# sara-nl/saraGAN

Measured on AMD Instinct MI355X. Metric: 3D volumes/sec/node (G+D step) at 128x128x32, higher is better.
Workload: dtype bf16

## Files before the change

### saragan_amd/csrc/common.h

```cpp
#pragma once
#include <hip/hip_runtime.h>
#include <stdint.h>
#include <mutex>
#include "../../include/saragan_hip.h"

typedef __bf16 bf16_t;
typedef float f32x4 __attribute__((ext_vector_type(4)));
typedef float f32x16 __attribute__((ext_vector_type(16)));
typedef __bf16 bf16x8 __attribute__((ext_vector_type(8)));
typedef __bf16 bf16x4 __attribute__((ext_vector_type(4)));
typedef short s16x4 __attribute__((ext_vector_type(4)));
typedef uint32_t u32x4 __attribute__((ext_vector_type(4)));

#define SG_STORE16_GUARD(v) asm volatile("s_nop 1" ::"v"(v))
typedef uint32_t u32x2 __attribute__((ext_vector_type(2)));

#define SG_LAUNCH_CHECK()                          \
  do {                                             \
    hipError_t e__ = hipGetLastError();            \
    if (e__ != hipSuccess) return (int)e__;        \
  } while (0)

static inline hipStream_t sg_st(sg_stream_t s) { return (hipStream_t)s; }

struct sg_config {
  int fwd_lds, fwd_tg;
  int fwd_v1, fwd_no_pw, fwd_no_dense;
  int fwd_no_v3, fwd_no_v3s, fwd_no_v4, fwd_no_v5, fwd_no_ksplit;
  int fwd3p_16;
  int fwd3s_16;
  int fwd_no_3p;
  int fwd3_gx, fwd3_no_lean;
  int fwd4_gx, fwd4_no_lean, fwd4_no_wres;
  int wgrad_v1, wgrad_no_v3, wgrad_no_lean;
  int wgrad_no_w16;
  int wgrad3l_min_cols;
  int wgrad3l_16;
  int wgrad_v1_blocks;
  int dbg_flags;
  int no_small;
  int deterministic;
  int gemm_ks_model;
  int gemm_k333_maxvox;
  int no_gemm;
};
const sg_config& sg_cfg();

bool sg_gemm_conv_eligible(const sg_conv_shape* s, sg_dtype dt);
size_t sg_gemm_conv_workspace(const sg_conv_shape* s, sg_dtype dt);
int sg_gemm_conv_fwd(const void* x, const void* wp, void* y, const sg_conv_shape* s, const float* bias, int act, float slope,
                     const uint32_t* mask_bits, float mask_slope, uint32_t* sign_out, void* workspace, size_t workspace_bytes,
                     hipStream_t st, bool* used);

bool sg_small_eligible(const sg_conv_shape* s);
bool sg_small_wgrad_eligible(const sg_conv_shape* s);
size_t sg_small_tail_bytes(const sg_conv_shape* s);
size_t sg_small_wgrad_workspace(const sg_conv_shape* s);
int sg_small_pack(const float* w, float coef, int flip, void* tail, const sg_conv_shape* s, sg_dtype dt, hipStream_t st);
int sg_small_fwd(const void* x, const void* tail, void* y, const sg_conv_shape* s, const float* bias, int act, float slope,
                 int pixel_norm, float eps, float* pn_scale, const uint32_t* mask_bits, float mask_slope, uint32_t* sign_out,
                 sg_dtype dt, hipStream_t st);
int sg_small_wgrad(const void* x, const void* dy, float* dw, float* dbias, float coef, void* workspace, size_t workspace_bytes,
// ... 259 lines not shown
```

### saragan_amd/csrc/conv3d.hip

```cpp
#include "common.h"
#include "prof.h"
#include "conv_args.h"

struct PackArgs {
  const float* w;
  void* wp;
  float coef;
  int taps, kd, kh, kw, cin, cout, nchunk, ntile, flip;
};

template <typename T>
__global__ void pack_weights_kernel(PackArgs a) {
  constexpr int CH = sg_traits<T>::CH;
  constexpr int EPL = CH / 2;
  const int64_t total = (int64_t)a.nchunk * a.taps * a.ntile * 64 * EPL;
  T* out = reinterpret_cast<T*>(a.wp);
  for (int64_t i = (int64_t)blockIdx.x * blockDim.x + threadIdx.x; i < total; i += (int64_t)gridDim.x * blockDim.x) {
    int e = (int)(i % EPL);
    int64_t q = i / EPL;
    int lane = (int)(q % 64); q /= 64;
    int nt = (int)(q % a.ntile); q /= a.ntile;
    int tap = (int)(q % a.taps);
    int chunk = (int)(q / a.taps);
    int ci = chunk * CH + (lane >> 5) * EPL + e;
// ... 29 lines not shown
    int lane = (int)(q % 64); q /= 64;
    int nt = (int)(q % a.ntile); q /= a.ntile;
    int tap = (int)(q % a.taps);
    int chunk = (int)(q / a.taps);
    int ci = chunk * CH + (lane >> 5) * EPL + e;
    int co = nt * 32 + (lane & 31);
    float v = 0.f;
    if (ci < a.cin && co < a.cout) {
      v = a.flip ? a.w[((int64_t)(a.taps - 1 - tap) * a.cout + co) * a.cin + ci] : a.w[((int64_t)tap * a.cin + ci) * a.cout + co];
      v *= a.coef;
    }
    out[i] = sg_traits<T>::from_f(v);
  }
}

static inline int conv_nchunk(const sg_conv_shape* s, sg_dtype dt) {
  int ch = dt == SG_BF16 ? 16 : 8;
  return sg_cdiv(s->cin, ch);
}
static inline int conv_ntile(const sg_conv_shape* s) { return sg_cdiv(s->cout, 32); }

static int conv_shape_ok(const sg_conv_shape* s) {
  if (!s) return 0;
  if (s->n < 1 || s->d < 1 || s->h < 1 || s->w < 1 || s->cin < 1 || s->cout < 1) return 0;
  const bool sub = s->kd == 2 && s->kh == 2 && s->kw == 2 && !s->upsample_in;
  if (s->kd < 1 || s->kh < 1 || s->kw < 1 || (!sub && (!(s->kd & 1) || !(s->kh & 1) || !(s->kw & 1)))) return 0;
  if (s->kd > 7 || s->kh > 7 || s->kw > 7) return 0;
  if (s->upsample_in && ((s->d | s->h | s->w) & 1)) return 0;
  return 1;
}

extern "C" size_t sg_conv3d_packed_bytes(const sg_conv_shape* s, sg_dtype dt) {
  if (!conv_shape_ok(s)) return 0;
  return (size_t)conv_nchunk(s, dt) * (s->kd * s->kh * s->kw) * conv_ntile(s) * 1024 + sg_small_tail_bytes(s) + sg_pack16_bytes(s, dt);
}

extern "C" int sg_conv3d_pack_weights(const float* w, float coef, int transpose_flip, void* wp,
                                      const sg_conv_shape* s, sg_dtype dt, sg_stream_t st) {
  if (!conv_shape_ok(s) || !w || !wp) return SG_EINVAL;
  PackArgs a;
  a.w = w; a.wp = wp; a.coef = coef;
  a.kd = s->kd; a.kh = s->kh; a.kw = s->kw; a.taps = s->kd * s->kh * s->kw;
  a.cin = s->cin; a.cout = s->cout; a.nchunk = conv_nchunk(s, dt); a.ntile = conv_ntile(s);
  a.flip = transpose_flip ? 1 : 0;
  int64_t total = (int64_t)a.nchunk * a.taps * a.ntile * 64 * (dt == SG_BF16 ? 8 : 4);
  int blocks = (int)((total + 255) / 256);
  if (blocks > 4096) blocks = 4096;
  if (dt == SG_BF16)
    hipLaunchKernelGGL(pack_weights_kernel<bf16_t>, dim3(blocks), dim3(256), 0, sg_st(st), a);
  else
    hipLaunchKernelGGL(pack_weights_kernel<float>, dim3(blocks), dim3(256), 0, sg_st(st), a);
  SG_LAUNCH_CHECK();
  if (sg_pack16_bytes(s, dt)) {
    void* tail = reinterpret_cast<char*>(wp) + (size_t)a.nchunk * a.taps * a.ntile * 1024;
    return sg_pack16_batch(1, &w, &coef, &a.flip, &tail, s, sg_st(st));
  }
  if (sg_small_tail_bytes(s))
    return sg_small_pack(w, coef, a.flip, reinterpret_cast<char*>(wp) + (size_t)a.nchunk * a.taps * a.ntile * 1024, s, dt, sg_st(st));
  return SG_OK;
}

extern "C" int sg_conv3d_pack_weights_batch(int n, const float* const* w, const float* coef, const int* transpose_flip,
                                            void* const* wp, const sg_conv_shape* shapes, sg_dtype dt, sg_stream_t st) {
  if (n < 0 || (n > 0 && (!w || !coef || !transpose_flip || !wp || !shapes))) return SG_EINVAL;
  if (dt != SG_BF16 && dt != SG_F32) return SG_EINVAL;
  for (int i = 0; i < n; ++i)
    if (!conv_shape_ok(&shapes[i]) || !w[i] || !wp[i]) return SG_EINVAL;
  for (int i0 = 0; i0 < n; i0 += SG_PACK_BATCH) {
    const int m = n - i0 < SG_PACK_BATCH ? n - i0 : SG_PACK_BATCH;
    PackBatchArgs b;
    int64_t most = 0;
    for (int j = 0; j < SG_PACK_BATCH; ++j) {
      const int i = i0 + (j < m ? j : 0);
      const sg_conv_shape* s = &shapes[i];
      PackArgs& a = b.item[j];
      a.w = w[i]; a.wp = wp[i]; a.coef = coef[i];
      a.kd = s->kd; a.kh = s->kh; a.kw = s->kw; a.taps = s->kd * s->kh * s->kw;
      a.cin = s->cin; a.cout = s->cout; a.nchunk = conv_nchunk(s, dt); a.ntile = conv_ntile(s);
      a.flip = transpose_flip[i] ? 1 : 0;
      const int64_t total = (int64_t)a.nchunk * a.taps * a.ntile * 64 * (dt == SG_BF16 ? 8 : 4);
      if (j < m && total > most) most = total;
    }
    int blocks = (int)((most + 255) / 256);
    if (blocks > 256) blocks = 256;
    if (blocks < 1) blocks = 1;
    if (dt == SG_BF16)
      hipLaunchKernelGGL(pack_weights_batch_kernel<bf16_t>, dim3((unsigned)blocks, (unsigned)m), dim3(256), 0, sg_st(st), b);
    else
      hipLaunchKernelGGL(pack_weights_batch_kernel<float>, dim3((unsigned)blocks, (unsigned)m), dim3(256), 0, sg_st(st), b);
    SG_LAUNCH_CHECK();
  }
  constexpr int M16 = 64;
  const float* w16[M16]; float c16[M16]; int f16[M16]; void* d16[M16]; sg_conv_shape s16[M16];
  int n16 = 0;
  for (int i = 0; i < n; ++i) {
    const sg_conv_shape* s = &shapes[i];
    char* tail = reinterpret_cast<char*>(wp[i]) + (size_t)conv_nchunk(s, dt) * (s->kd * s->kh * s->kw) * conv_ntile(s) * 1024;
    int rc = SG_OK;
    if (sg_pack16_bytes(s, dt)) {
      w16[n16] = w[i]; c16[n16] = coef[i]; f16[n16] = transpose_flip[i] ? 1 : 0; d16[n16] = tail; s16[n16] = *s;
      if (++n16 == M16) {
        rc = sg_pack16_batch(n16, w16, c16, f16, d16, s16, sg_st(st));
        n16 = 0;
      }
    } else if (sg_small_tail_bytes(s)) rc = sg_small_pack(w[i], coef[i], transpose_flip[i] ? 1 : 0, tail, s, dt, sg_st(st));
    if (rc != SG_OK) return rc;
  }
  if (n16) return sg_pack16_batch(n16, w16, c16, f16, d16, s16, sg_st(st));
  return SG_OK;
}


template <typename T> struct sg_vec4 { typedef u32x4 type; };
template <> struct sg_vec4<bf16_t> { typedef u32x2 type; };

template <typename T, int MTW, int NTB>
__device__ __forceinline__ void conv_epilogue(f32x16 (&acc)[MTW][NTB], const int64_t (&ooff)[MTW],
                                              const ConvFwdArgs& a, int nt0, int hh) {
  T* y = reinterpret_cast<T*>(a.y);
  const float inv_c = 1.f / (float)a.cout;
#pragma unroll
  for (int mt = 0; mt < MTW; ++mt) {
    float ss = 0.f;
#pragma unroll
    for (int nt = 0; nt < NTB; ++nt) {
#pragma unroll
      for (int i = 0; i < 16; ++i) {
        const int co = (nt0 + nt) * 32 + (i & 3) + 8 * (i >> 2) + 4 * hh;
        float v = acc[mt][nt][i];
        if (a.bias != nullptr && co < a.cout) v += a.bias[co];
        if (a.act) v = fmaxf(v, v * a.slope);
        acc[mt][nt][i] = v;
        ss += v * v;
      }
    }
    if (a.pixel_norm) {
      ss += __shfl_xor(ss, 32);
      const float sc = rsqrtf(ss * inv_c + a.eps);
#pragma unroll
      for (int nt = 0; nt < NTB; ++nt)
#pragma unroll
// ... 2098 lines not shown
    asm volatile("s_waitcnt vmcnt(0)" ::: "memory");
  };

  if (grp == 0) {
    init_acc();
    if (items_mine > 0 && ++cgS == ncg) { cgS = 0; ++kS; if (kS < kmine) enter_tile_S(); }
    for (int q = 0; q < items_max; ++q) {
      stamp();
      if (q < items_mine) mfma_phase(q);
      stamp();
      __syncthreads();
      stamp();
      off_phase(q < items_mine && (q % ncg) == ncg - 1, q + 1, q + 1, HF, NFRAG);
      stamp();
      __syncthreads();
    }
  } else {
    init_acc();
    for (int q = 0; q < items_max; ++q) {
      stamp();
      off_phase(q > 0 && q - 1 < items_mine && ((q - 1) % ncg) == ncg - 1, q, q + 1, 0, HF);
      stamp();
      __syncthreads();
      stamp();
      if (q < items_mine) mfma_phase(q);
      stamp();
      __syncthreads();
    }
    if (items_mine > 0 && items_mine == items_max) off_phase(true, items_mine, items_max, 0, 0);
    else if (items_mine > 0) {  }
  }
}

template <int EPI>
static int launch_fwd5_inst(const ConvFwdArgs& a, unsigned gx, unsigned gy, size_t lds, hipStream_t st) {
  auto kern = conv_fwd5_kernel<EPI>;
  SG_ALLOW_160K_LDS(kern);
  hipLaunchKernelGGL(kern, dim3(gx, gy), dim3(512), lds, st, a);
  return SG_OK;
}

static int launch_fwd5(ConvFwdArgs& a, const sg_conv_shape* s, hipStream_t st, bool* used) {
  *used = false;
  if (s->upsample_in || s->kd != 3 || s->kh != 3 || s->kw != 3 || a.os == 2 || a.tap_d || a.tap_h || a.tap_w) return SG_OK;
  if ((s->cin % 16) != 0 || (s->cout % 64) != 0 || a.pool == 1) return SG_OK;
  if (a.pool && ((s->h | s->w) & 1 || a.pixel_norm || a.mask_bits)) return SG_OK;
  if (a.pixel_norm && (a.mask_bits || a.ntile != 2)) return SG_OK;
  if (a.mask_bits && a.sign_out) return SG_OK;
  a.g = sg_make_geom(s, 256, true);
  const sg_tile_geom& g = a.g;
  if (g.TN != 1 || g.TW != 32 || (g.TH & 1) || g.TD * g.TH * g.TW != 256 || g.HD > 127 || g.HH > 127 || g.HW > 127) return SG_OK;
  const int64_t ntiles = (int64_t)g.nTn * g.nTd * g.nTh * g.nTw;
  const int ny = a.ntile / 2;
  int gx = (256 / ny) / 8 * 8;
  if (gx < 8) gx = 8;
  if (ntiles >= (1 << 24) || ntiles < 2 * gx) return SG_OK;
  {
    const int64_t svox = (int64_t)s->d * s->h * s->w;
    if (svox * s->cin * 2 >= (1ll << 31) || svox * s->cout * 2 >= (1ll << 31) || svox * a.ntile * 4 >= (1ll << 31)) return SG_OK;
  }
  const int hv = g.HD * g.HH * g.HW;
  if (sg_cdiv(hv * 2, 64) > 32) return SG_OK;
  a.G = 1;
  a.rs = 32;
  a.xbytes = hv * 32;
  a.wbytes = 27 * 2 * 1024;
  a.wres = 0;
  const size_t lds = 2ull * a.xbytes + 2ull * a.wbytes + 256;
  if (lds > 160 * 1024) return SG_OK;
  a.ntiles = (int)ntiles;
  a.vec_in = 1;
  a.vec_out = 1;
  const int epi = (a.sign_out ? SG_EP_SIGN : 0) | (a.mask_bits ? SG_EP_MASK : 0) | (a.pixel_norm ? SG_EP_PN : 0) |
                  (a.pool ? SG_EP_POOL : 0);
  int rc = SG_OK;
  switch (epi) {
    case 0: rc = launch_fwd5_inst<0>(a, (unsigned)gx, (unsigned)ny, lds, st); break;
    case SG_EP_POOL: rc = launch_fwd5_inst<SG_EP_POOL>(a, (unsigned)gx, (unsigned)ny, lds, st); break;
    case SG_EP_SIGN | SG_EP_POOL: rc = launch_fwd5_inst<SG_EP_SIGN | SG_EP_POOL>(a, (unsigned)gx, (unsigned)ny, lds, st); break;
    case SG_EP_SIGN: rc = launch_fwd5_inst<SG_EP_SIGN>(a, (unsigned)gx, (unsigned)ny, lds, st); break;
    case SG_EP_MASK: rc = launch_fwd5_inst<SG_EP_MASK>(a, (unsigned)gx, (unsigned)ny, lds, st); break;
    case SG_EP_PN: rc = launch_fwd5_inst<SG_EP_PN>(a, (unsigned)gx, (unsigned)ny, lds, st); break;
    case SG_EP_PN | SG_EP_SIGN: rc = launch_fwd5_inst<SG_EP_PN | SG_EP_SIGN>(a, (unsigned)gx, (unsigned)ny, lds, st); break;
    default: return SG_OK;
  }
  if (rc != SG_OK) return rc;
  SG_KNAME("conv_fwd5<bf16,2,2,3,3,3>");
  SG_LAUNCH_CHECK();
  *used = true;
  return SG_OK;
}

template <typename T>
__device__ __forceinline__ float sg_packed_w(const char* wp, int ntile, int cin_j, int cout_c) {
  constexpr int CH = sg_traits<T>::CH, ES = (int)sizeof(T);
  const int chunk = cin_j / CH, hh = (cin_j % CH) / (CH / 2), e = cin_j % (CH / 2);
  const char* frag = wp + ((int64_t)(chunk * ntile + (cout_c >> 5)) << 10);
  return sg_traits<T>::to_f(*reinterpret_cast<const T*>(frag + ((cout_c & 31) + 32 * hh) * 16 + e * ES));
}

template <typename T, int CIN>
__global__ __launch_bounds__(256) void pw_fwd_small_cin_kernel(ConvFwdArgs a, int64_t nvox) {
  constexpr int E = 16 / (int)sizeof(T);
  const int P = a.cout / E;
  const int p = threadIdx.x % P;
  const int c0 = p * E;
  const char* wp = reinterpret_cast<const char*>(a.wp);
  float w[CIN][E], b[E];
// ... 483 lines not shown
```

### saragan_amd/csrc/conv3w.hip

```cpp
#include "common.h"
#include "prof.h"
#include "conv_args.h"

typedef __attribute__((address_space(3))) void* lds_ptr3w_t;
typedef const __attribute__((address_space(1))) void* gbl_ptr3w_t;

namespace {

constexpr int W3_NFRAG = 54;
constexpr int W3_WBYTES = W3_NFRAG * 1024;
constexpr int W3_HROWS = 4 * 34;
constexpr int W3_HALO = W3_HROWS * 64;
constexpr int W3_HOFF = W3_WBYTES;
constexpr int W3_BOFF = W3_HOFF + 8 * W3_HALO;
constexpr int W3_POFF = W3_BOFF + 128;
constexpr int W3_MOFF = W3_POFF + 64;
constexpr int W3_AOFF = W3_MOFF + 128;
constexpr int W3_LDS = W3_MOFF + 128;
constexpr int W3_LDS_PWB = W3_AOFF + 8 * 4096;
static_assert(W3_LDS_PWB <= 160 * 1024, "LDS budget");
constexpr int W3_NPIECE = 9;
static_assert(W3_LDS <= 160 * 1024, "LDS budget");
#ifndef W3_PFW
#define W3_PFW 3
// ... 640 lines not shown
    if (E.j >= nitems) break;
    sg_kloop3w<2>::run(acc, xa, wl);
    stamp();
    SG_W3_OFF(2);
    if (E.j >= nitems) break;
  }
#undef SG_W3_OFF
  if constexpr (PWB) {
    const f32x4 fin[4] = {pwacc[0], pwacc[1], pwacc[2], pwacc[3]};
#pragma unroll
    for (int ch = 0; ch < 2; ++ch)
#pragma unroll
      for (int i = 0; i < 4; ++i) {
        float sw = fin[ch][i], sb = fin[2 + ch][i];
#pragma unroll
        for (int m = 1; m < 16; m <<= 1) {
          sw += __shfl_xor(sw, m);
          sb += __shfl_xor(sb, m);
        }
        if (v16 == 0) {
          float* row = a.pw_part + (size_t)(blockIdx.x * 8 + w8) * 64;
          row[16 * ch + 4 * q4 + i] = sw;
          row[32 + 16 * ch + 4 * q4 + i] = sb;
        }
      }
  }
}

struct Pack16Args {
  const float* w;
  bf16_t* out;
  float coef;
  int cin, cout, ngi, flip;
};
constexpr int SG_PACK16_BATCH = 32;
struct Pack16Batch {
  Pack16Args item[SG_PACK16_BATCH];
};
__global__ void pack_weights16_batch_kernel(Pack16Batch b) {
  const Pack16Args& a = b.item[blockIdx.y];
  const int ntile = a.cout >> 5;
  const int total = ntile * 27 * a.ngi * 2 * 64 * 8;
  for (int i = blockIdx.x * blockDim.x + threadIdx.x; i < total; i += gridDim.x * blockDim.x) {
    const int e = i & 7, lane = (i >> 3) & 63;
    int f = i >> 9;
    const int ch = f & 1;
    f >>= 1;
    const int gi = f % a.ngi;
    f /= a.ngi;
    const int tap = f % 27, nt = f / 27;
    const int co = 32 * nt + 16 * ch + (lane & 15), ci = 32 * gi + 8 * (lane >> 4) + e;
    const float v = !a.flip ? a.w[((int64_t)tap * a.cin + ci) * a.cout + co]
                            : a.w[((int64_t)(26 - tap) * a.cout + co) * a.cin + ci];
    a.out[i] = (bf16_t)(v * a.coef);
  }
}

__global__ __launch_bounds__(1024) void pw_part_final_kernel(const float* __restrict__ part, int rows, float* __restrict__ dw,
                                                             float* __restrict__ dbias, float coef) {
  __shared__ float red[16][64];
  const int col = threadIdx.x & 63, rg = threadIdx.x >> 6;
  float s8[8] = {0.f, 0.f, 0.f, 0.f, 0.f, 0.f, 0.f, 0.f};
  int b = rg;
  for (; b + 7 * 16 < rows; b += 8 * 16) {
#pragma unroll
    for (int u = 0; u < 8; ++u) s8[u] += part[(size_t)(b + u * 16) * 64 + col];
  }
  for (int u = 0; b < rows; b += 16, ++u) s8[u & 7] += part[(size_t)b * 64 + col];
  red[rg][col] = ((s8[0] + s8[1]) + (s8[2] + s8[3])) + ((s8[4] + s8[5]) + (s8[6] + s8[7]));
  __syncthreads();
  if (rg == 0) {
    float t = 0.f;
#pragma unroll
    for (int g = 0; g < 16; ++g) t += red[g][col];
    if (col < 32) { if (dw) dw[col] = coef * t; }
    else if (dbias) dbias[col - 32] = t;
  }
}

template <int EPI>
int launch_fwd3w_inst(const Fwd3wArgs& fa, unsigned gx, hipStream_t st) {
  auto kern = conv_fwd3w_kernel<EPI>;
  SG_ALLOW_160K_LDS(kern);
  hipLaunchKernelGGL(kern, dim3(gx, (unsigned)fa.a.ntile), dim3(512), (EPI & SG_EP_PWB) ? W3_LDS_PWB : W3_LDS, st, fa);
  return SG_OK;
}

}

size_t sg_pack16_bytes(const sg_conv_shape* s, sg_dtype dt) {
  if (dt != SG_BF16 || s->kd != 3 || s->kh != 3 || s->kw != 3 || (s->cout & 31) || s->cout < 32) return 0;
  if (!((s->cin == 64 && s->cout == 32) || s->cin == 32)) return 0;
  return (size_t)(s->cout >> 5) * 27 * (s->cin >> 5) * 2 * 1024;
}

int sg_pack16_batch(int n, const float* const* w, const float* coef, const int* flip, void* const* dst, const sg_conv_shape* shapes,
                    hipStream_t st) {
  for (int i0 = 0; i0 < n; i0 += SG_PACK16_BATCH) {
    const int m = n - i0 < SG_PACK16_BATCH ? n - i0 : SG_PACK16_BATCH;
    Pack16Batch b;
    for (int j = 0; j < SG_PACK16_BATCH; ++j) {
      const int i = i0 + (j < m ? j : 0);
      Pack16Args& p = b.item[j];
      p.w = w[i]; p.out = reinterpret_cast<bf16_t*>(dst[i]); p.coef = coef[i];
      p.cin = shapes[i].cin; p.cout = shapes[i].cout; p.ngi = shapes[i].cin >> 5; p.flip = flip[i] ? 1 : 0;
    }
    hipLaunchKernelGGL(pack_weights16_batch_kernel, dim3(54, (unsigned)m), dim3(256), 0, st, b);
    SG_LAUNCH_CHECK();
  }
  return SG_OK;
}

int sg_pw_wgrad_finalize(const float* part, int rows, float* dw, float* dbias, float coef, hipStream_t st) {
  if (!dw && !dbias) return SG_OK;
  hipLaunchKernelGGL(pw_part_final_kernel, dim3(1), dim3(1024), 0, st, part, rows, dw, dbias, coef);
  SG_LAUNCH_CHECK();
  return SG_OK;
}

int sg_launch_fwd3w(ConvFwdArgs& a, const sg_conv_shape* s, hipStream_t st, bool* used, int* pw_rows) {
  *used = false;
  *pw_rows = 0;
  if (s->kd != 3 || s->kh != 3 || s->kw != 3 || s->cin != 32 || (s->cout & 31) || a.xcs != 32 || a.xco != 0) return SG_OK;
  if (s->upsample_in || a.in_mask || a.addend) return SG_OK;
  if (s->d < 2 || s->h < 8 || (s->w % 32) != 0) return SG_OK;
  if (a.pool && ((a.pool != 1 && a.pool != 3) || (s->d & 1) || (a.pool == 3 && ((s->h | s->w) & 1)) || a.pixel_norm || a.pnb_y || (a.mask_bits && (a.sign_out || a.bias || a.act)))) return SG_OK;
  if (a.pixel_norm && (a.mask_bits || a.ntile != 1 || a.pnb_y)) return SG_OK;
  if (a.mask_bits && a.sign_out) return SG_OK;
  if (a.pnb_y && (a.ntile != 1 || !a.mask_bits || a.sign_out || a.bias || a.act || !a.pnb_scale)) return SG_OK;
  if (a.rgb_out && (a.ntile != 1 || !a.rgb_w || a.pool || a.mask_bits || a.pnb_y || !a.pixel_norm || !a.sign_out)) return SG_OK;
  if (a.pw_x && (a.ntile != 1 || !a.pw_wmat || !a.pw_part || !a.mask_bits || a.pool || a.pnb_y || a.rgb_out || a.pixel_norm ||
                 a.sign_out || a.bias || a.act)) return SG_OK;
  {
    const int64_t svox = (int64_t)s->d * s->h * s->w;
    if (svox * 64 >= (1ll << 31) || svox * s->cout * 2 >= (1ll << 31) || svox * a.ntile * 4 >= (1ll << 31)) return SG_OK;
  }
  Fwd3wArgs fa;
  fa.a = a;
// ... 50 lines not shown
```

### saragan_amd/csrc/conv_args.h

```cpp
#pragma once
#include "common.h"

struct ConvFwdArgs {
  const void* x;
  const void* wp;
  void* y;
  const float* bias;
  float* pn_scale;
  const uint32_t* mask_bits;
  uint32_t* sign_out;
  float mask_slope;
  sg_tile_geom g;
  int cin, cout, taps, kh, kw;
  int nchunk, ntile;
  int G, TG;
  int rs;
  int xbytes;
  sg_fastdiv fnp;
  int sshift, rshift;
  int wbytes, ntiles;
  int wres;
  int lean;
  int tap_d, tap_h, tap_w;
  int xcs, xco;
  const float* addend;
  const void* pnb_y;
  const float* pnb_scale;
  const uint32_t* in_mask;
  float in_mask_slope, in_gain;
  int in_mask_nw;
  const float* rgb_w;
  const float* rgb_bias;
  void* rgb_out;
  const void* pw_x;
  const float* pw_wmat;
  void* pw_dx;
  float* pw_part;
  int pool;
  int os, oa, ob, oc;
  unsigned long long* dbg;
  int dbg_flags;
  int vec_in, vec_out;
  int act, pixel_norm;
  float slope, eps;
};

enum : int { SG_EP_SIGN = 1, SG_EP_MASK = 2, SG_EP_PN = 4, SG_EP_POOL = 8, SG_EP_PNB = 16,
              SG_EP_RGB = 32, SG_EP_PWB = 128, SG_EP_POOL3 = 256   };

int sg_launch_fwd3p(ConvFwdArgs& a, const sg_conv_shape* s, hipStream_t st, bool* used);
int sg_launch_fwd3w(ConvFwdArgs& a, const sg_conv_shape* s, hipStream_t st, bool* used, int* pw_rows);
constexpr int SG_PW_PART_ROWS = 2048;
int sg_pw_wgrad_finalize(const float* part, int rows, float* dw, float* dbias, float coef, hipStream_t st);
size_t sg_pack16_bytes(const sg_conv_shape* s, sg_dtype dt);
int sg_pack16_batch(int n, const float* const* w, const float* coef, const int* flip, void* const* dst, const sg_conv_shape* shapes,
                    hipStream_t st);
```

### saragan_amd/csrc/prof.hip

```cpp
#include "prof.h"
#include <mutex>
#include <vector>
#include <string.h>
#include <stdlib.h>
#include <atomic>

namespace {
struct Rec { int kind; sg_conv_shape shape; int dtype; hipEvent_t e0, e1; bool ok; const char* name; };
std::mutex g_mu;
bool g_on = false;
bool g_filter = false;
int g_fkind = 0;
sg_conv_shape g_fshape;
std::vector<Rec> g_recs;
const char* kVersion = "saragan_hip 0.4 (gfx950)";
}

bool sg_prof_on() { return g_on; }
thread_local const char* sg_tls_kernel = "";

namespace {
std::atomic<const sg_config*> g_cfg{nullptr};
int env_int(const char* name, int dflt) {
  const char* v = getenv(name);
  return v && *v ? atoi(v) : dflt;
}
const sg_config* read_config() {
  sg_config* c = new sg_config;
  c->fwd_lds = env_int("SG_FWD_LDS", 80 * 1024);
  c->fwd_tg = env_int("SG_FWD_TG", 0);
  c->fwd_v1 = env_int("SG_FWD_V1", 0);
  c->fwd_no_pw = env_int("SG_FWD_NO_PW", 0);
  c->fwd_no_dense = env_int("SG_FWD_NO_DENSE", 0);
  c->fwd_no_v3 = env_int("SG_FWD_NO_V3", 0);
  c->fwd_no_v3s = env_int("SG_FWD_NO_V3S", 0);
  c->wgrad_no_lean = env_int("SG_WGRAD_NO_LEAN", 0);
  c->wgrad_no_w16 = env_int("SG_WGRAD_NO_W16", 0);
  c->wgrad3l_16 = env_int("SG_WGRAD3L_16", 0);
  c->wgrad3l_min_cols = env_int("SG_WGRAD3L_MIN_COLS", 0);
  c->wgrad_v1_blocks = env_int("SG_WGRAD_V1_BLOCKS", 0);
  c->fwd_no_v4 = env_int("SG_FWD_NO_V4", 0);
  c->fwd_no_v5 = env_int("SG_FWD_NO_V5", 0);
  c->fwd_no_ksplit = env_int("SG_FWD_NO_KSPLIT", 0);
  c->fwd_no_3p = env_int("SG_FWD_NO_3P", 0);
  c->fwd3p_16 = env_int("SG_FWD3P_16", 1);
  c->fwd3s_16 = env_int("SG_FWD3S_16", 1);
  c->fwd3_gx = env_int("SG_FWD3_GX", 0);
  c->fwd3_no_lean = env_int("SG_FWD3_NO_LEAN", 0);
  c->fwd4_gx = env_int("SG_FWD4_GX", 0);
  c->fwd4_no_lean = env_int("SG_FWD4_NO_LEAN", 0);
  c->fwd4_no_wres = env_int("SG_FWD4_NO_WRES", 0);
  c->wgrad_v1 = env_int("SG_WGRAD_V1", 0);
  c->wgrad_no_v3 = env_int("SG_WGRAD_NO_V3", 0);
  c->dbg_flags = env_int("SG_DBG_FLAGS", 0);
  c->no_small = env_int("SG_NO_SMALL", 0);
  c->deterministic = env_int("SG_DETERMINISTIC", 0);
  c->no_gemm = env_int("SG_NO_GEMM", 0);
  c->gemm_ks_model = env_int("SG_GEMM_KS_MODEL", 0);
  c->gemm_k333_maxvox = env_int("SG_GEMM_K333_MAXVOX", 8192);
  return c;
}
}

const sg_config& sg_cfg() {
  const sg_config* c = g_cfg.load(std::memory_order_acquire);
  if (c == nullptr) {
    std::lock_guard<std::mutex> lk(g_mu);
    c = g_cfg.load(std::memory_order_acquire);
    if (c == nullptr) {
      c = read_config();
      g_cfg.store(c, std::memory_order_release);
    }
  }
  return *c;
}

extern "C" int sg_config_reload(void) {
  std::lock_guard<std::mutex> lk(g_mu);
// ... 96 lines not shown
```

Before: 615.1.

## Add fwd5p conv kernel using 16x16x32 bf16 MFMA with new packed weight layout

Adds a new 3x3x3 forward convolution kernel variant (fwd5p) that uses v_mfma_f32_16x16x32_bf16 with a fully unrolled, statically checked LDS-read/MFMA schedule, and pairs taps so that 27 taps map to 13 pairs plus a tail. A new weight packing format (kind 1) is added to the batch packing kernel and stored after the pack16 tail, and the packed buffer size grows to hold it. By default (SG_FWD5_16=1) the new kernel replaces fwd5 for eligible shapes without pixel norm, with the aim of raising MFMA throughput and reducing LDS traffic. This adds extra weight packing work and storage, and a complex hand-scheduled kernel whose lgkmcnt accounting is fragile.

Result: no change. 620.6 (median of 6 runs) (+0.9%).

```diff
diff --git a/saragan_amd/csrc/common.h b/saragan_amd/csrc/common.h
--- a/saragan_amd/csrc/common.h
+++ b/saragan_amd/csrc/common.h
@@ -28,6 +28,7 @@
   int fwd_v1, fwd_no_pw, fwd_no_dense;
   int fwd_no_v3, fwd_no_v3s, fwd_no_v4, fwd_no_v5, fwd_no_ksplit;
   int fwd3p_16;
+  int fwd5_16;
   int fwd3s_16;
   int fwd_no_3p;
   int fwd3_gx, fwd3_no_lean;
diff --git a/saragan_amd/csrc/conv3d.hip b/saragan_amd/csrc/conv3d.hip
--- a/saragan_amd/csrc/conv3d.hip
+++ b/saragan_amd/csrc/conv3d.hip
@@ -85,7 +85,8 @@
 
 extern "C" size_t sg_conv3d_packed_bytes(const sg_conv_shape* s, sg_dtype dt) {
   if (!conv_shape_ok(s)) return 0;
-  return (size_t)conv_nchunk(s, dt) * (s->kd * s->kh * s->kw) * conv_ntile(s) * 1024 + sg_small_tail_bytes(s) + sg_pack16_bytes(s, dt);
+  return (size_t)conv_nchunk(s, dt) * (s->kd * s->kh * s->kw) * conv_ntile(s) * 1024 + sg_small_tail_bytes(s) + sg_pack16_bytes(s, dt) +
+         sg_pack5_bytes(s, dt);
 }
 
 extern "C" int sg_conv3d_pack_weights(const float* w, float coef, int transpose_flip, void* wp,
@@ -104,9 +105,17 @@
   else
     hipLaunchKernelGGL(pack_weights_kernel<float>, dim3(blocks), dim3(256), 0, sg_st(st), a);
   SG_LAUNCH_CHECK();
-  if (sg_pack16_bytes(s, dt)) {
-    void* tail = reinterpret_cast<char*>(wp) + (size_t)a.nchunk * a.taps * a.ntile * 1024;
-    return sg_pack16_batch(1, &w, &coef, &a.flip, &tail, s, sg_st(st));
+  if (sg_pack16_bytes(s, dt) || sg_pack5_bytes(s, dt)) {
+    char* tail = reinterpret_cast<char*>(wp) + (size_t)a.nchunk * a.taps * a.ntile * 1024;
+    const float* w2[2] = {w, w};
+    const float c2[2] = {coef, coef};
+    const int f2[2] = {a.flip, a.flip};
+    const sg_conv_shape s2[2] = {*s, *s};
+    void* d2[2];
+    int k2[2], m = 0;
+    if (sg_pack16_bytes(s, dt)) { d2[m] = tail; k2[m++] = 0; }
+    if (sg_pack5_bytes(s, dt)) { d2[m] = tail + sg_pack16_bytes(s, dt); k2[m++] = 1; }
+    return sg_pack16_batch(m, w2, c2, f2, d2, s2, k2, sg_st(st));
   }
   if (sg_small_tail_bytes(s))
     return sg_small_pack(w, coef, a.flip, reinterpret_cast<char*>(wp) + (size_t)a.nchunk * a.taps * a.ntile * 1024, s, dt, sg_st(st));
@@ -143,23 +152,29 @@
       hipLaunchKernelGGL(pack_weights_batch_kernel<float>, dim3((unsigned)blocks, (unsigned)m), dim3(256), 0, sg_st(st), b);
     SG_LAUNCH_CHECK();
   }
-  constexpr int M16 = 64;
-  const float* w16[M16]; float c16[M16]; int f16[M16]; void* d16[M16]; sg_conv_shape s16[M16];
+  constexpr int M16 = 80;
+  const float* w16[M16]; float c16[M16]; int f16[M16]; void* d16[M16]; sg_conv_shape s16[M16]; int k16[M16];
   int n16 = 0;
   for (int i = 0; i < n; ++i) {
     const sg_conv_shape* s = &shapes[i];
     char* tail = reinterpret_cast<char*>(wp[i]) + (size_t)conv_nchunk(s, dt) * (s->kd * s->kh * s->kw) * conv_ntile(s) * 1024;
     int rc = SG_OK;
-    if (sg_pack16_bytes(s, dt)) {
-      w16[n16] = w[i]; c16[n16] = coef[i]; f16[n16] = transpose_flip[i] ? 1 : 0; d16[n16] = tail; s16[n16] = *s;
-      if (++n16 == M16) {
-        rc = sg_pack16_batch(n16, w16, c16, f16, d16, s16, sg_st(st));
-        n16 = 0;
+    const size_t b16 = sg_pack16_bytes(s, dt), b5 = sg_pack5_bytes(s, dt);
+    if (b16 || b5) {
+      for (int kind = 0; kind < 2; ++kind) {
+        if (!(kind ? b5 : b16)) continue;
+        w16[n16] = w[i]; c16[n16] = coef[i]; f16[n16] = transpose_flip[i] ? 1 : 0; d16[n16] = tail + (kind ? b16 : 0); s16[n16] = *s;
+        k16[n16] = kind;
+        if (++n16 == M16) {
+          rc = sg_pack16_batch(n16, w16, c16, f16, d16, s16, k16, sg_st(st));
+          n16 = 0;
+          if (rc != SG_OK) return rc;
+        }
       }
     } else if (sg_small_tail_bytes(s)) rc = sg_small_pack(w[i], coef[i], transpose_flip[i] ? 1 : 0, tail, s, dt, sg_st(st));
     if (rc != SG_OK) return rc;
   }
-  if (n16) return sg_pack16_batch(n16, w16, c16, f16, d16, s16, sg_st(st));
+  if (n16) return sg_pack16_batch(n16, w16, c16, f16, d16, s16, k16, sg_st(st));
   return SG_OK;
 }
 
@@ -2324,6 +2339,415 @@
   }
 }
 
+struct sg_unrolled_k5p {
+  static constexpr int NS = 14, NR = 8;
+  static constexpr int need(int m) { return 4 + m / 4; }
+  static constexpr int issued_next(int s, int m) { return s + 1 < NS ? (m == 0 ? 0 : m == 1 ? 2 : 4) + m / 4 : 0; }
+  static constexpr bool waits(int m) { return (m & 3) == 0; }
+  static constexpr int younger(int s, int m) { return NR - 1 - need(m) + issued_next(s, m); }
+  static constexpr bool counts_ok() {
+    for (int s = 0; s < NS; ++s)
+      for (int m = 0; m < 16; ++m) if (younger(s, m) < 0 || younger(s, m) > 15) return false;
+    return younger(0, 0) == 3 && younger(0, 4) == 7 && younger(0, 12) == 7 && younger(NS - 1, 12) == 0;
+  }
+  static constexpr int NA = 30;
+
+  template <int S, int B>
+  static __device__ __forceinline__ void rdb(u32x4 (&bfr)[2][4], const int (&xa)[NA]) {
+    if constexpr (S < NS - 1)
+      asm volatile("ds_read_b128 %0, %1 offset:%2" : "=v"(bfr[S & 1][B]) : "v"(xa[2 * S + (B >> 1)]), "n"((B & 1) * 512));
+    else
+      asm volatile("ds_read_b128 %0, %1" : "=v"(bfr[S & 1][B]) : "v"(xa[26 + B]));
+  }
+  template <int S, int CG>
+  static __device__ __forceinline__ void rda(u32x4 (&afr)[4], int wl, int wlh) {
+    if constexpr (S < NS - 1)
+      asm volatile("ds_read_b128 %0, %1 offset:%2" : "=v"(afr[CG]) : "v"(wl), "n"((S * 4 + CG) << 10));
+    else
+      asm volatile("ds_read_b128 %0, %1 offset:%2" : "=v"(afr[CG]) : "v"(wlh), "n"(((NS - 1) * 4 << 10) + CG * 512));
+  }
+  static __device__ __forceinline__ void mfma(f32x4& c, const u32x4& a_, const u32x4& b_) {
+    asm volatile("v_mfma_f32_16x16x32_bf16 %0, %1, %2, %0" : "+v"(c) : "v"(a_), "v"(b_));
+  }
+  template <int S, int M>
+  static __device__ __forceinline__ void step(f32x4 (&acc)[2][2][4], u32x4 (&afr)[4], u32x4 (&bfr)[2][4], const int (&xa)[NA], int wl,
+                                              int wlh) {
+    if constexpr (S < NS) {
+      if constexpr (waits(M)) {
+        SG_WAIT_LGKM(younger(S, M));
+        __builtin_amdgcn_sched_barrier(0);
+      }
+      mfma(acc[(M >> 1) & 1][M & 1][M >> 2], afr[M >> 2], bfr[S & 1][M & 3]);
+      if constexpr (S + 1 < NS) {
+        if constexpr (M < 2) {
+          rdb<S + 1, 2 * M>(bfr, xa);
+          rdb<S + 1, 2 * M + 1>(bfr, xa);
+        }
+        if constexpr ((M & 3) == 3) rda<S + 1, (M >> 2)>(afr, wl, wlh);
+      }
+      if constexpr (M < 15) step<S, M + 1>(acc, afr, bfr, xa, wl, wlh);
+      else step<S + 1, 0>(acc, afr, bfr, xa, wl, wlh);
+    }
+  }
+  static __device__ __forceinline__ void run(f32x4 (&acc)[2][2][4], const int (&xa)[NA], int wl, int wlh) {
+    u32x4 afr[4], bfr[2][4];
+    SG_KLOOP_BEGIN();
+    rdb<0, 0>(bfr, xa); rdb<0, 1>(bfr, xa); rdb<0, 2>(bfr, xa); rdb<0, 3>(bfr, xa);
+    rda<0, 0>(afr, wl, wlh); rda<0, 1>(afr, wl, wlh); rda<0, 2>(afr, wl, wlh); rda<0, 3>(afr, wl, wlh);
+    step<0, 0>(acc, afr, bfr, xa, wl, wlh);
+    asm volatile("s_nop 7\n\ts_nop 7\n\ts_nop 3"
+                 : "+v"(acc[0][0][0]), "+v"(acc[0][0][1]), "+v"(acc[0][0][2]), "+v"(acc[0][0][3]),
+                   "+v"(acc[0][1][0]), "+v"(acc[0][1][1]), "+v"(acc[0][1][2]), "+v"(acc[0][1][3]),
+                   "+v"(acc[1][0][0]), "+v"(acc[1][0][1]), "+v"(acc[1][0][2]), "+v"(acc[1][0][3]),
+                   "+v"(acc[1][1][0]), "+v"(acc[1][1][1]), "+v"(acc[1][1][2]), "+v"(acc[1][1][3]));
+    SG_KLOOP_END();
+  }
+};
+static_assert(sg_unrolled_k5p::counts_ok(), "a needed read is issued too late, or lgkmcnt (a 4-bit counter) would overflow");
+
+template <int EPI>
+__global__ __launch_bounds__(512) void conv_fwd5p_kernel(ConvFwdArgs a) {
+  extern __shared__ __attribute__((aligned(16))) char smem[];
+  constexpr int ES = 2, EPP = 8, NFRAG = 54, HF = NFRAG / 2;
+  constexpr uint32_t DEAD = 0x80000000u;
+  constexpr bool SIGN = (EPI & SG_EP_SIGN) != 0, MASK = (EPI & SG_EP_MASK) != 0, PN = (EPI & SG_EP_PN) != 0;
+  constexpr bool POOL = (EPI & SG_EP_POOL) != 0;
+  const sg_tile_geom& g = a.g;
+  const int tid = threadIdx.x, lane = tid & 63;
+  const int wave8 = __builtin_amdgcn_readfirstlane(tid >> 6);
+  const int grp = wave8 >> 2, wave = wave8 & 3;
+  const int q4 = lane >> 4, v16 = (lane & 15) ^ ((lane & 8) ? 0 : 4);
+  const int xmine = grp * a.xbytes, wbase = 2 * a.xbytes;
+  float* bias_lds = reinterpret_cast<float*>(smem + 2 * a.xbytes + 2 * a.wbytes);
+  const int zoff = 2 * a.xbytes + 2 * a.wbytes + 256;
+  const int nt0 = blockIdx.y * 2;
+  const int ncg = a.nchunk, cout = a.cout, ntile = a.ntile, cin = a.cin;
+  const int D = g.D, H = g.H, W = g.W;
+
+  const int xg = blockIdx.x & 7, slot = blockIdx.x >> 3;
+  const int per_x = gridDim.x >> 3;
+  const int cpx = (a.ntiles + 7) >> 3;
+  const int t_begin = xg * cpx;
+  const int t_end = min(a.ntiles, t_begin + cpx);
+  const int first = t_begin + slot;
+  const int K = first < t_end ? (t_end - first + per_x - 1) / per_x : 0;
+  const int kmine = (K + 1 - grp) >> 1;
+  const int items_mine = kmine * ncg;
+  const int items_max = ((K + 1) >> 1) * ncg;
+
+  int xa[sg_unrolled_k5p::NA];
+  int tcoord[2];
+  {
+    const int tsel = q4 >> 1, half = q4 & 1;
+#pragma unroll
+    for (int mt = 0; mt < 2; ++mt) {
+      const int q = wave * 2 + mt;
+      const int th = q % g.TH, td = q / g.TH;
+      tcoord[mt] = (th << 8) | (td << 16);
+      const int lrow = (td * g.HH + th) * g.HW + v16;
+      auto addr_of = [&](int row) { return xmine + row * 32 + ((half ^ ((row >> 3) & 1)) << 4); };
+      auto shift_of = [&](int t) { return ((t / 9) * g.HH + (t / 3) % 3) * g.HW + t % 3; };
+#pragma unroll
+      for (int p = 0; p < 13; ++p) xa[2 * p + mt] = addr_of(lrow + (tsel ? shift_of(2 * p + 1) : shift_of(2 * p)));
+#pragma unroll
+      for (int vh = 0; vh < 2; ++vh) xa[26 + 2 * mt + vh] = tsel ? zoff : addr_of(lrow + shift_of(26) + 16 * vh);
+    }
+  }
+  const int hv = g.HD * g.HH * g.HW;
+  constexpr int MAXIT = 8;
+  uint32_t relb[MAXIT];
+  int crd[MAXIT];
+#pragma unroll
+  for (int k = 0; k < MAXIT; ++k) {
+    const int it = (wave + 4 * k) * 64 + lane;
+    const int row = it >> 1;
+    const int sl = (it & 1) ^ ((row >> 3) & 1);
+    uint32_t q = sg_div((uint32_t)row, g.fHW);
+    const int hw = (int)(row - q * g.HW);
+    uint32_t q2 = sg_div(q, g.fHH);
+    const int hh_ = (int)(q - q2 * g.HH), hd = (int)q2;
+    relb[k] = row < hv ? (uint32_t)((((hd * H + hh_) * W + hw) * cin + sl * EPP) * ES) : 0xC0000000u;
+    crd[k] = row < hv ? (hw | (hh_ << 8) | (hd << 16)) : 0x7F7F7F7F;
+  }
+  const int64_t svox = (int64_t)D * H * W;
+  const int64_t xsb = svox * cin * ES, ysb = (POOL ? svox >> 2 : svox) * cout * ES, wsb = svox * ntile * 4, psb = svox * 4;
+  auto rsrc_of = [&](const void* base, int64_t sample_bytes, int n0) {
+    return __builtin_amdgcn_make_buffer_rsrc(const_cast<char*>(reinterpret_cast<const char*>(base)) + n0 * sample_bytes, 0,
+                                             (int)sample_bytes, 0x00020000);
+  };
+  const __amdgpu_buffer_rsrc_t rw = __builtin_amdgcn_make_buffer_rsrc(const_cast<void*>(a.wp), 0, 0x7FFFFFFF, 0x00020000);
+
+  int kS = 0, cgS = 0;
+  __amdgpu_buffer_rsrc_t rxS;
+  uint32_t vk[MAXIT];
+  auto enter_tile_S = [&]() {
+    const sg_tile_origin o = sg_tile_of(g, (uint32_t)(first + (2 * kS + grp) * per_x));
+    rxS = rsrc_of(a.x, xsb, o.n0);
+    const int tile_off = (((o.d0 - 1) * H + (o.h0 - 1)) * W + (o.w0 - 1)) * cin * ES;
+    const int lo_w = max(0, 1 - o.w0), hi_w = min(g.HW, W + 1 - o.w0) - 1;
+    const int lo_h = max(0, 1 - o.h0), hi_h = min(g.HH, H + 1 - o.h0) - 1;
+    const int lo_d = max(0, 1 - o.d0), hi_d = min(g.HD, D + 1 - o.d0) - 1;
+    const uint32_t lo = (uint32_t)(lo_w | (lo_h << 8) | (lo_d << 16));
+    const uint32_t hi = (uint32_t)(hi_w | (hi_h << 8) | (hi_d << 16)) | 0x808080u;
+#pragma unroll
+    for (int k = 0; k < MAXIT; ++k) {
+      const uint32_t c_ = (uint32_t)crd[k] & 0xFFFFFFu;
+      const uint32_t t1 = (c_ | 0x808080u) - lo, t2 = hi - c_;
+      vk[k] = (t1 & t2 & 0x808080u) == 0x808080u ? relb[k] + (uint32_t)tile_off : DEAD;
+    }
+  };
+  auto stage_halo = [&]() {
+    const uint32_t soff = (uint32_t)(cgS * 32);
+#pragma unroll
+    for (int k = 0; k < MAXIT; ++k)
+      if ((wave + 4 * k) * 64 < hv * 2 && crd[k] != 0x7F7F7F7F)
+        __builtin_amdgcn_raw_ptr_buffer_load_lds(rxS, (lds_ptr_t)(smem + xmine + (wave + 4 * k) * 1024), 16, vk[k], soff, 0, 0);
+  };
+  auto stage_slab = [&](int j, int f0, int f1, int w, int nw) {
+    const int cg = j % ncg;
+    char* dst = smem + wbase + (j & 1) * a.wbytes;
+    const uint32_t cbase = (uint32_t)((cg * (int)gridDim.y + (int)blockIdx.y) * NFRAG) << 10;
+    for (int f = f0 + w; f < f1; f += nw)
+      __builtin_amdgcn_raw_ptr_buffer_load_lds(rw, (lds_ptr_t)(dst + (f << 10)), 16, (uint32_t)(lane * 16), cbase + ((uint32_t)f << 10), 0, 0);
+  };
+  int kE = 0;
+  __amdgpu_buffer_rsrc_t ryE, rsE, rmE, rpE;
+  uint32_t vox[2][2];
+  uint32_t pvox = DEAD;
+  auto enter_tile_E = [&]() {
+    const sg_tile_origin o = sg_tile_of(g, (uint32_t)(first + (2 * kE + grp) * per_x));
+    ryE = rsrc_of(a.y, ysb, o.n0);
+    if (SIGN) rsE = rsrc_of(a.sign_out, wsb, o.n0);
+    if (MASK) rmE = rsrc_of(a.mask_bits, wsb, o.n0);
+    if (PN) rpE = rsrc_of(a.pn_scale, psb, o.n0);
+#pragma unroll
+    for (int mt = 0; mt < 2; ++mt) {
+      const int tc = tcoord[mt];
+      const int d = o.d0 + (tc >> 16), h = o.h0 + ((tc >> 8) & 255);
+#pragma unroll
+      for (int vh = 0; vh < 2; ++vh) {
+        const int w = o.w0 + 16 * vh + v16;
+        vox[mt][vh] = (d < D && h < H && w < W) ? (uint32_t)((d * H + h) * W + w) : DEAD;
+      }
+      if (POOL && mt == 0) {
+        const int w = o.w0 + 2 * ((v16 >> 1) + 8 * (v16 & 1));
+        pvox = (d < D && h < H && w < W) ? (uint32_t)((d * (H >> 1) + (h >> 1)) * (W >> 1) + (w >> 1)) : DEAD;
+      }
+    }
+  };
+  uint32_t mbn[2][2][2] = {{{0u, 0u}, {0u, 0u}}, {{0u, 0u}, {0u, 0u}}};
+  auto request_mask = [&]() {
+    if constexpr (MASK) {
+#pragma unroll
+      for (int mt = 0; mt < 2; ++mt)
+#pragma unroll
+        for (int vh = 0; vh < 2; ++vh)
+#pragma unroll
+          for (int nt = 0; nt < 2; ++nt)
+            mbn[mt][vh][nt] = __builtin_amdgcn_raw_buffer_load_b32(rmE, (kE < kmine && vox[mt][vh] != DEAD) ? (vox[mt][vh] * (uint32_t)ntile + nt0 + nt) * 4u : DEAD, 0, 0);
+    }
+  };
+
+  if (tid < 64) {
+    const int co = nt0 * 32 + tid;
+    bias_lds[tid] = (a.bias != nullptr && co < cout) ? a.bias[co] : 0.f;
+  } else if (tid < 68) {
+    reinterpret_cast<uint32_t*>(smem + zoff)[tid - 64] = 0u;
+  }
+  if (items_max > 0) stage_slab(0, 0, NFRAG, wave8, 8);
+  if (items_mine > 0) {
+    enter_tile_S();
+    enter_tile_E();
+    request_mask();
+    if (grp == 0) stage_halo();
+  }
+  asm volatile("s_waitcnt vmcnt(0)" ::: "memory");
+  __syncthreads();
+
+  const int wl0 = wbase + lane * 16, wlh0 = wbase + (lane & 31) * 16;
+  const float inv_c = 1.f / (float)cout;
+  const float slope = a.act ? a.slope : 1.f;
+  const uint32_t cb = (uint32_t)((q4 & 1) * 16 + (q4 >> 1) * 8);
+  f32x4 acc[2][2][4];
+  auto init_acc = [&]() {
+#pragma unroll
+    for (int cg = 0; cg < 4; ++cg) {
+      const f32x4 b4 = *reinterpret_cast<const f32x4*>(bias_lds + cg * 16 + 4 * q4);
+#pragma unroll
+      for (int mt = 0; mt < 2; ++mt)
+#pragma unroll
+        for (int vh = 0; vh < 2; ++vh) acc[mt][vh][cg] = b4;
+    }
+    asm volatile("" : "+v"(acc[0][0][0]), "+v"(acc[0][0][1]), "+v"(acc[0][0][2]), "+v"(acc[0][0][3]),
+                      "+v"(acc[0][1][0]), "+v"(acc[0][1][1]), "+v"(acc[0][1][2]), "+v"(acc[0][1][3]),
+                      "+v"(acc[1][0][0]), "+v"(acc[1][0][1]), "+v"(acc[1][0][2]), "+v"(acc[1][0][3]),
+                      "+v"(acc[1][1][0]), "+v"(acc[1][1][1]), "+v"(acc[1][1][2]), "+v"(acc[1][1][3]));
+  };
+  int dbgi = 0;
+  auto stamp = [&]() {
+    if (a.dbg != nullptr && blockIdx.x == 8 && blockIdx.y == 0 && lane == 0 && wave == 0 && dbgi < 120)
+      a.dbg[grp * 128 + dbgi] = __builtin_amdgcn_s_memtime();
+    ++dbgi;
+  };
+  auto mfma_phase = [&](int q) { sg_unrolled_k5p::run(acc, xa, wl0 + (q & 1) * a.wbytes, wlh0 + (q & 1) * a.wbytes); };
+  auto quad_sum = [](float v) {
+    const auto r1 = __builtin_amdgcn_permlane16_swap(__float_as_uint(v), __float_as_uint(v), false, false);
+    const float s1 = __uint_as_float(r1[0]) + __uint_as_float(r1[1]);
+    const auto r2 = __builtin_amdgcn_permlane32_swap(__float_as_uint(s1), __float_as_uint(s1), false, false);
+    return __uint_as_float(r2[0]) + __uint_as_float(r2[1]);
+  };
+  auto store_tile = [&](const float (&lo)[4], const float (&hi)[4], const __amdgpu_buffer_rsrc_t& rs, uint32_t voff) {
+    const uint32_t a0 = sg_pack_bf16(lo[0], lo[1]), a1 = sg_pack_bf16(lo[2], lo[3]);
+    const uint32_t b0 = sg_pack_bf16(hi[0], hi[1]), b1 = sg_pack_bf16(hi[2], hi[3]);
+    const auto s0 = __builtin_amdgcn_permlane16_swap(a0, b0, false, false);
+    const auto s1 = __builtin_amdgcn_permlane16_swap(a1, b1, false, false);
+    u32x4 out;
+    out[0] = s0[0]; out[1] = s1[0]; out[2] = s0[1]; out[3] = s1[1];
+    __builtin_amdgcn_raw_buffer_store_b128(out, rs, voff, 0, 0);
+    SG_STORE16_GUARD(out);
+  };
+
+  auto off_phase = [&](bool closes, int qn, int js, int f0, int f1) {
+    if (qn < items_mine) stage_halo();
+    if (js < items_max) stage_slab(js, f0, f1, wave, 4);
+    __builtin_amdgcn_sched_barrier(0);
+    stamp();
+    if (closes) {
+      uint32_t part[2][4] = {{0u, 0u, 0u, 0u}, {0u, 0u, 0u, 0u}};
+#pragma unroll
+      for (int mt = 0; mt < 2; ++mt)
+#pragma unroll
+        for (int vh = 0; vh < 2; ++vh) {
+          f32x4(&t)[4] = acc[mt][vh];
+          const bool ok = vox[mt][vh] != DEAD;
+          if (slope != 1.f) {
+#pragma unroll
+            for (int cg = 0; cg < 4; ++cg)
+#pragma unroll
+              for (int i = 0; i < 4; ++i) t[cg][i] = sg_lrelu(t[cg][i], slope);
+          }
+          if (PN) {
+            float ss = 0.f;
+#pragma unroll
+            for (int cg = 0; cg < 4; ++cg)
+#pragma unroll
+              for (int i = 0; i < 4; ++i) ss += t[cg][i] * t[cg][i];
+            ss = quad_sum(ss);
+            const float sc = rsqrtf(ss * inv_c + a.eps);
+#pragma unroll
+            for (int cg = 0; cg < 4; ++cg)
+#pragma unroll
+              for (int i = 0; i < 4; ++i) t[cg][i] *= sc;
+            if (a.pn_scale != nullptr)
+              __builtin_amdgcn_raw_buffer_store_b32(__float_as_uint(sc), rpE, (ok && q4 == 0) ? vox[mt][vh] * 4u : DEAD, 0, 0);
+          }
+#pragma unroll
+          for (int nt = 0; nt < 2; ++nt) {
+            if (SIGN) {
+              uint32_t b = 0u;
+#pragma unroll
+              for (int ch = 0; ch < 2; ++ch)
+#pragma unroll
+                for (int i = 0; i < 4; ++i) b |= (__float_as_uint(t[2 * nt + ch][i]) >> 31) << (16 * ch + i);
+              part[nt][2 * mt + vh] = b << (4 * q4);
+            }
+            if (MASK) {
+              const uint32_t wsh = mbn[mt][vh][nt] >> (4 * q4);
+              const float sm1 = a.mask_slope - 1.f;
+#pragma unroll
+              for (int ch = 0; ch < 2; ++ch)
+#pragma unroll
+                for (int i = 0; i < 4; ++i) {
+                  const int t_ = ((int)(wsh << (31 - (16 * ch + i)))) >> 31;
+                  t[2 * nt + ch][i] += __uint_as_float((uint32_t)t_ & __float_as_uint(t[2 * nt + ch][i] * sm1));
+                }
+            }
+            if constexpr (!POOL) {
+              const float lo[4] = {t[2 * nt][0], t[2 * nt][1], t[2 * nt][2], t[2 * nt][3]};
+              const float hi[4] = {t[2 * nt + 1][0], t[2 * nt + 1][1], t[2 * nt + 1][2], t[2 * nt + 1][3]};
+              store_tile(lo, hi, ryE, ok ? (vox[mt][vh] * (uint32_t)cout + (uint32_t)((nt0 + nt) * 32) + cb) * 2u : DEAD);
+            }
+          }
+        }
+      if constexpr (SIGN) {
+        const uint32_t sv = q4 == 0 ? vox[0][0] : q4 == 1 ? vox[0][1] : q4 == 2 ? vox[1][0] : vox[1][1];
+#pragma unroll
+        for (int nt = 0; nt < 2; ++nt) {
+          const auto r01 = __builtin_amdgcn_permlane16_swap(part[nt][0], part[nt][1], false, false);
+          const auto r23 = __builtin_amdgcn_permlane16_swap(part[nt][2], part[nt][3], false, false);
+          const auto rr = __builtin_amdgcn_permlane32_swap(r01[0] | r01[1], r23[0] | r23[1], false, false);
+          __builtin_amdgcn_raw_buffer_store_b32(rr[0] | rr[1], rsE, sv != DEAD ? (sv * (uint32_t)ntile + nt0 + nt) * 4u : DEAD, 0, 0);
+        }
+      }
+      if constexpr (POOL) {
+#pragma unroll
+        for (int nt = 0; nt < 2; ++nt) {
+          float m[2][4];
+#pragma unroll
+          for (int ch = 0; ch < 2; ++ch)
+#pragma unroll
+            for (int i = 0; i < 4; ++i) {
+              const float c0 = acc[0][0][2 * nt + ch][i] + acc[1][0][2 * nt + ch][i];
+              const float c1 = acc[0][1][2 * nt + ch][i] + acc[1][1][2 * nt + ch][i];
+              const float u0 = c0 + __uint_as_float((uint32_t)__builtin_amdgcn_update_dpp(0, (int)__float_as_uint(c0), 0xB1, 0xF, 0xF, true));
+              const float u1 = c1 + __uint_as_float((uint32_t)__builtin_amdgcn_update_dpp(0, (int)__float_as_uint(c1), 0xB1, 0xF, 0xF, true));
+              m[ch][i] = ((v16 & 1) ? u1 : u0) * 0.25f;
+            }
+          store_tile(m[0], m[1], ryE, pvox != DEAD ? (pvox * (uint32_t)cout + (uint32_t)((nt0 + nt) * 32) + cb) * 2u : DEAD);
+        }
+      }
+      ++kE;
+      if (kE < kmine) enter_tile_E();
+      request_mask();
+      init_acc();
+    }
+    if (qn < items_mine) {
+      if (++cgS == ncg) {
+        cgS = 0;
+        ++kS;
+        if (kS < kmine) enter_tile_S();
+      }
+    }
+    asm volatile("s_waitcnt vmcnt(0)" ::: "memory");
+  };
+
+  if (grp == 0) {
+    init_acc();
+    if (items_mine > 0 && ++cgS == ncg) { cgS = 0; ++kS; if (kS < kmine) enter_tile_S(); }
+    for (int q = 0; q < items_max; ++q) {
+      stamp();
+      if (q < items_mine) mfma_phase(q);
+      stamp();
+      __syncthreads();
+      stamp();
+      off_phase(q < items_mine && (q % ncg) == ncg - 1, q + 1, q + 1, HF, NFRAG);
+      stamp();
+      __syncthreads();
+    }
+  } else {
+    init_acc();
+    for (int q = 0; q < items_max; ++q) {
+      stamp();
+      off_phase(q > 0 && q - 1 < items_mine && ((q - 1) % ncg) == ncg - 1, q, q + 1, 0, HF);
+      stamp();
+      __syncthreads();
+      stamp();
+      if (q < items_mine) mfma_phase(q);
+      stamp();
+      __syncthreads();
+    }
+    if (items_mine > 0 && items_mine == items_max) off_phase(true, items_mine, items_max, 0, 0);
+  }
+}
+
+template <int EPI>
+static int launch_fwd5p_inst(const ConvFwdArgs& a, unsigned gx, unsigned gy, size_t lds, hipStream_t st) {
+  auto kern = conv_fwd5p_kernel<EPI>;
+  SG_ALLOW_160K_LDS(kern);
+  hipLaunchKernelGGL(kern, dim3(gx, gy), dim3(512), lds, st, a);
+  return SG_OK;
+}
+
 template <int EPI>
 static int launch_fwd5_inst(const ConvFwdArgs& a, unsigned gx, unsigned gy, size_t lds, hipStream_t st) {
   auto kern = conv_fwd5_kernel<EPI>;
@@ -2366,6 +2790,22 @@
   const int epi = (a.sign_out ? SG_EP_SIGN : 0) | (a.mask_bits ? SG_EP_MASK : 0) | (a.pixel_norm ? SG_EP_PN : 0) |
                   (a.pool ? SG_EP_POOL : 0);
   int rc = SG_OK;
+  const size_t lds16 = lds + 16;
+  const bool use16 = sg_cfg().fwd5_16 == 2 || (sg_cfg().fwd5_16 == 1 && !a.pixel_norm);
+  if (use16 && sg_pack5_bytes(s, SG_BF16) && lds16 <= 160 * 1024) {
+    ConvFwdArgs b = a;
+    b.wp = reinterpret_cast<const char*>(a.wp) + (size_t)a.nchunk * a.taps * a.ntile * 1024 + sg_pack16_bytes(s, SG_BF16);
+    switch (epi) {
+      case 0: rc = launch_fwd5p_inst<0>(b, (unsigned)gx, (unsigned)ny, lds16, st); break;
+      case SG_EP_POOL: rc = launch_fwd5p_inst<SG_EP_POOL>(b, (unsigned)gx, (unsigned)ny, lds16, st); break;
+      case SG_EP_SIGN | SG_EP_POOL: rc = launch_fwd5p_inst<SG_EP_SIGN | SG_EP_POOL>(b, (unsigned)gx, (unsigned)ny, lds16, st); break;
+      case SG_EP_SIGN: rc = launch_fwd5p_inst<SG_EP_SIGN>(b, (unsigned)gx, (unsigned)ny, lds16, st); break;
+      case SG_EP_MASK: rc = launch_fwd5p_inst<SG_EP_MASK>(b, (unsigned)gx, (unsigned)ny, lds16, st); break;
+      case SG_EP_PN: rc = launch_fwd5p_inst<SG_EP_PN>(b, (unsigned)gx, (unsigned)ny, lds16, st); break;
+      case SG_EP_PN | SG_EP_SIGN: rc = launch_fwd5p_inst<SG_EP_PN | SG_EP_SIGN>(b, (unsigned)gx, (unsigned)ny, lds16, st); break;
+      default: return SG_OK;
+    }
+  } else
   switch (epi) {
     case 0: rc = launch_fwd5_inst<0>(a, (unsigned)gx, (unsigned)ny, lds, st); break;
     case SG_EP_POOL: rc = launch_fwd5_inst<SG_EP_POOL>(a, (unsigned)gx, (unsigned)ny, lds, st); break;
diff --git a/saragan_amd/csrc/conv3w.hip b/saragan_amd/csrc/conv3w.hip
--- a/saragan_amd/csrc/conv3w.hip
+++ b/saragan_amd/csrc/conv3w.hip
@@ -696,13 +696,41 @@
   bf16_t* out;
   float coef;
   int cin, cout, ngi, flip;
+  int kind;
 };
-constexpr int SG_PACK16_BATCH = 32;
+constexpr int SG_PACK16_BATCH = 80;
 struct Pack16Batch {
   Pack16Args item[SG_PACK16_BATCH];
 };
+static_assert(sizeof(Pack16Batch) <= 4096, "kernel arguments");
+constexpr int SG_PACK5_PAIRS = 13, SG_PACK5_SLAB = SG_PACK5_PAIRS * 4 * 512 + 4 * 256;
 __global__ void pack_weights16_batch_kernel(Pack16Batch b) {
   const Pack16Args& a = b.item[blockIdx.y];
+  if (a.kind == 1) {
+    const int nb = a.cout >> 6;
+    const int total = (a.cin >> 4) * nb * SG_PACK5_SLAB;
+    for (int i = blockIdx.x * blockDim.x + threadIdx.x; i < total; i += gridDim.x * blockDim.x) {
+      const int slab = i / SG_PACK5_SLAB, r = i - slab * SG_PACK5_SLAB;
+      const int chunk = slab / nb, blk = slab - chunk * nb;
+      const int e = r & 7;
+      int lane, cg, tap;
+      if (r < SG_PACK5_PAIRS * 4 * 512) {
+        lane = (r >> 3) & 63;
+        cg = (r >> 9) & 3;
+        tap = 2 * (r >> 11) + (lane >> 5);
+      } else {
+        const int r2 = r - SG_PACK5_PAIRS * 4 * 512;
+        lane = (r2 >> 3) & 31;
+        cg = r2 >> 8;
+        tap = 26;
+      }
+      const int co = 64 * blk + 16 * cg + (lane & 15), ci = 16 * chunk + 8 * ((lane >> 4) & 1) + e;
+      const float v = !a.flip ? a.w[((int64_t)tap * a.cin + ci) * a.cout + co]
+                              : a.w[((int64_t)(26 - tap) * a.cout + co) * a.cin + ci];
+      a.out[i] = (bf16_t)(v * a.coef);
+    }
+    return;
+  }
   const int ntile = a.cout >> 5;
   const int total = ntile * 27 * a.ngi * 2 * 64 * 8;
   for (int i = blockIdx.x * blockDim.x + threadIdx.x; i < total; i += gridDim.x * blockDim.x) {
@@ -758,8 +786,14 @@
   return (size_t)(s->cout >> 5) * 27 * (s->cin >> 5) * 2 * 1024;
 }
 
+size_t sg_pack5_bytes(const sg_conv_shape* s, sg_dtype dt) {
+  if (dt != SG_BF16 || s->kd != 3 || s->kh != 3 || s->kw != 3 || (s->cin & 15) || (s->cout & 63)) return 0;
+  if (s->cin * s->cout > 128 * 128) return 0;
+  return (size_t)(s->cin >> 4) * (s->cout >> 6) * SG_PACK5_SLAB * sizeof(bf16_t);
+}
+
 int sg_pack16_batch(int n, const float* const* w, const float* coef, const int* flip, void* const* dst, const sg_conv_shape* shapes,
-                    hipStream_t st) {
+                    const int* kind, hipStream_t st) {
   for (int i0 = 0; i0 < n; i0 += SG_PACK16_BATCH) {
     const int m = n - i0 < SG_PACK16_BATCH ? n - i0 : SG_PACK16_BATCH;
     Pack16Batch b;
@@ -767,7 +801,7 @@
       const int i = i0 + (j < m ? j : 0);
       Pack16Args& p = b.item[j];
       p.w = w[i]; p.out = reinterpret_cast<bf16_t*>(dst[i]); p.coef = coef[i];
-      p.cin = shapes[i].cin; p.cout = shapes[i].cout; p.ngi = shapes[i].cin >> 5; p.flip = flip[i] ? 1 : 0;
+      p.cin = shapes[i].cin; p.cout = shapes[i].cout; p.ngi = shapes[i].cin >> 5; p.flip = flip[i] ? 1 : 0; p.kind = kind[i];
     }
     hipLaunchKernelGGL(pack_weights16_batch_kernel, dim3(54, (unsigned)m), dim3(256), 0, st, b);
     SG_LAUNCH_CHECK();
diff --git a/saragan_amd/csrc/conv_args.h b/saragan_amd/csrc/conv_args.h
--- a/saragan_amd/csrc/conv_args.h
+++ b/saragan_amd/csrc/conv_args.h
@@ -53,5 +53,6 @@
 constexpr int SG_PW_PART_ROWS = 2048;
 int sg_pw_wgrad_finalize(const float* part, int rows, float* dw, float* dbias, float coef, hipStream_t st);
 size_t sg_pack16_bytes(const sg_conv_shape* s, sg_dtype dt);
+size_t sg_pack5_bytes(const sg_conv_shape* s, sg_dtype dt);
 int sg_pack16_batch(int n, const float* const* w, const float* coef, const int* flip, void* const* dst, const sg_conv_shape* shapes,
-                    hipStream_t st);
+                    const int* kind, hipStream_t st);
diff --git a/saragan_amd/csrc/prof.hip b/saragan_amd/csrc/prof.hip
--- a/saragan_amd/csrc/prof.hip
+++ b/saragan_amd/csrc/prof.hip
@@ -44,6 +44,7 @@
   c->fwd_no_ksplit = env_int("SG_FWD_NO_KSPLIT", 0);
   c->fwd_no_3p = env_int("SG_FWD_NO_3P", 0);
   c->fwd3p_16 = env_int("SG_FWD3P_16", 1);
+  c->fwd5_16 = env_int("SG_FWD5_16", 1);
   c->fwd3s_16 = env_int("SG_FWD3S_16", 1);
   c->fwd3_gx = env_int("SG_FWD3_GX", 0);
   c->fwd3_no_lean = env_int("SG_FWD3_NO_LEAN", 0);
```
